# SensorsINI/v2e

Hardware: NVIDIA H100
Metric: Mevents/s (higher is better)
Workload: dtype fp16 tensor-core convs (fp32 accumulate) + f64 pixel state

## Files before the change

### include/v2e_b200.h

```cpp
#ifndef V2E_B200_H
#define V2E_B200_H

#include <stdint.h>

#ifdef __cplusplus
extern "C" {
#endif

typedef enum V2eStatus {
    V2E_OK = 0,
    V2E_E_INVALID = -1,
    V2E_E_CUDA = -2,
    V2E_E_CAPACITY = -3,
    V2E_E_ITER_CAP = -4,
    V2E_E_STATE = -5,
    V2E_E_UNSUPPORTED = -6,
    V2E_E_FALLBACK = -7
} V2eStatus;

typedef enum V2eFrameDtype { V2E_U8 = 0, V2E_F32 = 1, V2E_F64 = 2 } V2eFrameDtype;

const char *v2e_last_error(void);
int v2e_version(void);
int v2e_abi_info(int *version, int *emu_cfg_size, int *frame_info_size, int *unet_weights_size);
// ... 139 lines not shown
int v2e_conv2d_lrelu_sm100(const void *x1_dev, int C1, const void *x2_dev, int C2,
                           const void *wgt_dev, const float *bias_dev, int Cout_pad, int KH, int KW,
                           int N, int H, int W, void *out_dev, int out_cstride, int out_mode,
                           int co_real, float slope, void *stream);

enum {
    V2E_CONV_TILE_AUTO = -1,
    V2E_CONV_TILE_LEGACY = 0,
    V2E_CONV_TILE_256x128 = 1,
    V2E_CONV_TILE_128x256 = 2
};
int v2e_conv2d_lrelu_sm100_tile(const void *x1_dev, int C1, const void *x2_dev, int C2,
                                const void *wgt_dev, const float *bias_dev, int Cout_pad, int KH, int KW,
                                int N, int H, int W, void *out_dev, int out_cstride, int out_mode,
                                int co_real, float slope, int tile, void *stream);
int v2e_conv_pick_tile(int C1, int C2, int Cout_pad, int KH, int KW, int N, int H, int W, int n_sms);

int v2e_conv2d_lrelu_sm100_strip(const void *x1_dev, int C1, const void *x2_dev, int C2,
                                 const void *wgt_row_dev, const float *bias_dev, int Cout_pad, int KH,
                                 int KW, int N, int H, int W, void *out_dev, int out_cstride,
                                 int out_mode, int co_real, float slope, void *stream);
int v2e_conv_strip_pick_kc(int C1, int C2, int Cout_pad, int KH, int KW, int W);

int v2e_conv2d_up2_lrelu_sm100(const void *x_low_dev, int C, const void *wgt_fold_dev, const void *wgt_plain_dev,
                               const float *bias_dev, int Cout_pad, int N, int H_out, int W_out, void *out_dev,
                               int out_cstride, float slope, void *stream);
int v2e_conv_up2_fold_weights(const float *w_host, int cout, int cin, int Cout_pad, int C_pad, void *out_host);
int v2e_conv_up2_supported_c(int C, int Cout_pad, int W_out);

typedef struct V2eUNetWeights {
    const float *w[23];
    const float *b[23];
} V2eUNetWeights;

typedef struct V2eSlomo V2eSlomo;

int v2e_slomo_create(int H, int W, int max_batch, const V2eUNetWeights *flow,
                     const V2eUNetWeights *interp, V2eSlomo **out);
int v2e_slomo_destroy(V2eSlomo *h);
int v2e_slomo_set_pairs(V2eSlomo *h, const uint8_t *frames_u8_dev, int B, void *stream);
int v2e_slomo_max_flow(V2eSlomo *h, float *max_speed_host, void *stream);
int v2e_slomo_interp(V2eSlomo *h, double t, uint8_t *out_u8_dev, float *out_f32_dev, void *stream);
int v2e_slomo_check_finite(V2eSlomo *h, int *nonfinite_host, void *stream);
int v2e_slomo_set_option(V2eSlomo *h, int option, int value);
int v2e_slomo_profile(V2eSlomo *h, int enable);
int v2e_slomo_profile_read(V2eSlomo *h, float *conv_ms, int *conv_launches, double *conv_flops, void *stream);
// ... 70 lines not shown
```

### v2e_b200/_lib.py

```python
import ctypes
import os

from . import build as _build

_LIB = None


class V2eEmuCfg(ctypes.Structure):
    _fields_ = [
        ("width", ctypes.c_int32), ("height", ctypes.c_int32),
        ("per_pixel_thres", ctypes.c_int32), ("hdr", ctypes.c_int32),
        ("pos_thres_nominal", ctypes.c_double), ("neg_thres_nominal", ctypes.c_double),
        ("cutoff_hz", ctypes.c_double), ("leak_rate_hz", ctypes.c_double),
        ("leak_jitter_fraction", ctypes.c_double), ("refractory_period_s", ctypes.c_double),
        ("shot_noise_rate_hz", ctypes.c_double), ("shot_inten_factor", ctypes.c_double),
        ("rng_mode", ctypes.c_int32), ("iter_cap", ctypes.c_int32),
        ("seed", ctypes.c_uint64),
        ("csdvs", ctypes.c_int32), ("max_frames_per_step", ctypes.c_int32),
        ("cs_tau_p_s", ctypes.c_double), ("cs_tau_h_s", ctypes.c_double),
        ("scidvs", ctypes.c_int32), ("photoreceptor_noise", ctypes.c_int32),
        ("rng_pixel_offset", ctypes.c_uint32), ("full_frame_px", ctypes.c_uint32),
        ("own_row0", ctypes.c_int32), ("own_rows", ctypes.c_int32),
        ("cs_halo_rows", ctypes.c_int32), ("reserved1", ctypes.c_int32),
    ]
# ... 57 lines not shown
    "v2e_emu_phase_count": (_i, [_vp, _vp, _i, _d, _d, _vp, _vp, _i, _u64, _u64, _vp]),
    "v2e_emu_phase_update": (_i, [_vp, _vp, _i, _d, _d, _vp, _vp, _u64, _u64, _vp]),
    "v2e_emu_max_n_dev": (_vp, [_vp]),
    "v2e_emu_cs_begin": (_i, [_vp, _vp, _i, _d, _d, _u64, _u64, ctypes.POINTER(_i), _vp]),
    "v2e_emu_cs_pack": (_i, [_vp, _vp]),
    "v2e_emu_cs_unpack_from": (_i, [_vp, _vp, _vp, _vp]),
    "v2e_emu_cs_send_dev": (_vp, [_vp]),
    "v2e_emu_cs_chunk": (_i, [_vp, _i, _i, _vp]),
    "v2e_emu_cs_max_dev": (_vp, [_vp]),
    "v2e_emu_cs_advance": (_i, [_vp, _i, _i, _vp]),
    "v2e_emu_cs_update": (_i, [_vp, _vp, _i, _vp, _vp, _vp]),
    "v2e_emu_phase_filter": (_i, [_vp, _d, _d, _u64, _i, _vp]),
    "v2e_emu_read_counts": (_i, [_vp, ctypes.POINTER(ctypes.c_int32), _vp, _i, _vp]),
    "v2e_emu_phase_shot": (_i, [_vp, _vp, _i, _d, _d, _vp, _u64, _vp]),
    "v2e_emu_phase_emit": (_i, [_vp, _d, _d, _vp, _u64, _vp]),
    "v2e_conv2d_lrelu_sm100": (_i, [_vp, _i, _vp, _i, _vp, _vp, _i, _i, _i, _i, _i, _i, _vp, _i, _i, _i,
                                    ctypes.c_float, _vp]),
    "v2e_conv2d_lrelu_sm100_tile": (_i, [_vp, _i, _vp, _i, _vp, _vp, _i, _i, _i, _i, _i, _i, _vp, _i, _i, _i,
                                         ctypes.c_float, _i, _vp]),
    "v2e_conv_pick_tile": (_i, [_i, _i, _i, _i, _i, _i, _i, _i, _i]),
    "v2e_conv2d_lrelu_sm100_strip": (_i, [_vp, _i, _vp, _i, _vp, _vp, _i, _i, _i, _i, _i, _i, _vp, _i, _i, _i,
                                          ctypes.c_float, _vp]),
    "v2e_conv_strip_pick_kc": (_i, [_i, _i, _i, _i, _i, _i]),
    "v2e_conv2d_up2_lrelu_sm100": (_i, [_vp, _i, _vp, _vp, _vp, _i, _i, _i, _i, _vp, _i, ctypes.c_float, _vp]),
    "v2e_conv_up2_fold_weights": (_i, [_vp, _i, _i, _i, _i, _vp]),
    "v2e_conv_up2_supported_c": (_i, [_i, _i, _i]),
    "v2e_slomo_create": (_i, [_i, _i, _i, _vp, _vp, ctypes.POINTER(_vp)]),
    "v2e_slomo_destroy": (_i, [_vp]),
    "v2e_slomo_set_pairs": (_i, [_vp, _vp, _i, _vp]),
    "v2e_slomo_max_flow": (_i, [_vp, ctypes.POINTER(ctypes.c_float), _vp]),
    "v2e_slomo_interp": (_i, [_vp, _d, _vp, _vp, _vp]),
    "v2e_slomo_set_option": (_i, [_vp, _i, _i]),
    "v2e_slomo_check_finite": (_i, [_vp, ctypes.POINTER(_i), _vp]),
    "v2e_slomo_profile": (_i, [_vp, _i]),
    "v2e_slomo_profile_read": (_i, [_vp, ctypes.POINTER(ctypes.c_float), ctypes.POINTER(_i),
                                    ctypes.POINTER(ctypes.c_double), _vp]),
    "v2e_slomo_profile_read_layers": (_i, [_vp, ctypes.POINTER(ctypes.c_float), ctypes.POINTER(_i),
                                           ctypes.POINTER(ctypes.c_double), ctypes.POINTER(ctypes.c_float),
                                           ctypes.POINTER(_i), ctypes.POINTER(ctypes.c_double), _vp]),
    "v2e_slomo_flow_ptr": (_vp, [_vp]),
    "v2e_slomo_intrp_ptr": (_vp, [_vp]),
    "v2e_slomo_buffer_ptr": (_vp, [_vp, _i, _i]),
    "v2e_slomo_layer_kernel": (_i, [_vp, _i, _i]),
    "v2e_resize_create": (_i, [_i, _i, _i, _i, _i, _i, ctypes.POINTER(_vp)]),
    "v2e_resize_destroy": (_i, [_vp]),
    "v2e_resize_run": (_i, [_vp, _vp, _vp, _i, _vp]),
# ... 91 lines not shown
```

### v2e_b200/csrc/conv_tc.cu

```cuda
#include <cuda.h>
#include <cuda_fp16.h>
#include <cuda_runtime.h>
#include <math.h>
#include <stdint.h>
#include <stdio.h>
#include <string.h>
#include <vector>

#include "../../include/v2e_b200.h"
#include "common.cuh"
#include "tc_common.cuh"

namespace {

constexpr int kTileH = 8, kTileW = 16, kBM = kTileH * kTileW;
constexpr int kStages = 4;
constexpr int kConvThreads = 288;
constexpr int kProducerWarp = 8;
constexpr int kConsumerWarps = 8;

struct ConvParams {
    int N, H, W;
    int C1, C2;
    int KH, KW;
// ... 255 lines not shown
constexpr int kStripThreads = 288;

struct RowRing {
    uint64_t *full, *empty;
    uint32_t nslot, cnt;
    int waited, released;
    __device__ __forceinline__ uint32_t slot(int i) const { return (cnt + (uint32_t)i) % nslot; }
    __device__ __forceinline__ void wait_upto(int n) {
        for (; waited < n; waited++) {
            const uint32_t g = cnt + (uint32_t)waited;
            mbar_wait(&full[g % nslot], (g / nslot) & 1u);
        }
    }
    __device__ __forceinline__ void release_upto(int n, int lane) {
        wait_upto(n);
        __syncwarp();
        for (; released < n; released++)
            if (lane == 0) mbar_arrive(&empty[slot(released)]);
    }
};

template <int KW, int KC, int BN>
__device__ __forceinline__ void strip_pair_mma(float (&acc)[2][BN / 2], const RowRing &rr, int row0, int last, int slabs,
                                               uint64_t dr, uint64_t dw, uint32_t a_off, uint32_t row16, uint32_t slab16) {
    constexpr int KH = KW, taps = KH * KW;
    constexpr uint32_t rowb16 = (KC * 2u) >> 4, tile16 = (BN * KC * 2u) >> 4;
#pragma unroll
    for (int k = 0; k < 2; k++) {
#pragma unroll
        for (int i = 0; i < BN / 2; i++) acc[k][i] = 0.f;
        wgmma_fence_regs(acc[k]);
    }
    wgmma_fence();
#pragma unroll
    for (int rp = 0; rp <= KH; rp++) {
        const uint32_t a_row = rr.slot(row0 + (rp < KH ? rp : last)) * row16 + a_off;
        int sl = 0;
#pragma unroll 1
        do {
            const uint32_t a_lo = a_row + (uint32_t)sl * slab16;
#pragma unroll
            for (int s = 0; s < KW; s++) {
#pragma unroll
                for (int j = 0; j < KC / 16; j++) {
                    const uint64_t ad = desc_add(dr, a_lo + (uint32_t)s * rowb16 + 2u * j);
                    if (rp < KH) wgmma_f16<BN>(acc[0], ad, desc_add(dw, (uint32_t)(sl * taps + rp * KW + s) * tile16 + 2u * j), 1u);
                    if (rp > 0) wgmma_f16<BN>(acc[1], ad, desc_add(dw, (uint32_t)(sl * taps + (rp - 1) * KW + s) * tile16 + 2u * j), 1u);
                }
            }
        } while (++sl < slabs);
    }
    wgmma_commit();
}

template <int KW, int KC, int BN, bool POOL>
__global__ void __launch_bounds__(kStripThreads, 1)
conv_strip_kernel(const __grid_constant__ CUtensorMap tmA, const __grid_constant__ CUtensorMap tmA2,
                  const __grid_constant__ CUtensorMap tmB, const StripParams p) {
    extern __shared__ __align__(1024) uint8_t smem_raw[];
    uint8_t *smem = align1024(smem_raw);
    __shared__ __align__(8) uint64_t full_bar[kMaxSlot], empty_bar[kMaxSlot], w_bar;

    constexpr int KH = KW, ph = KH / 2, pw = KW / 2, taps = KH * KW;
    constexpr int PW = kRowTile + KW - 1;
    constexpr uint32_t tile_bytes = BN * KC * 2;
    const int warp = threadIdx.x >> 5, lane = threadIdx.x & 31;
    const int slabs = (p.C1 + p.C2) / KC;
    const uint32_t row_bytes = (uint32_t)p.slab_bytes * slabs;
    uint8_t *ring = smem + ((p.w_bytes + 1023) & ~1023);
    const int split = (int)blockIdx.x % p.n_split, co_off = split * BN;
    const int item0 = (int)blockIdx.x / p.n_split, item_step = (int)gridDim.x / p.n_split;

    if (threadIdx.x == 0) {
        for (int s = 0; s < p.nslot; s++) { mbar_init(&full_bar[s], 1); mbar_init(&empty_bar[s], kConsumerWarps); }
        mbar_init(&w_bar, 1);
        fence_barrier_init();
    }
    if (warp == kProducerWarp && lane == 0) {
        prefetch_tmap(&tmA);
        if (p.C2) prefetch_tmap(&tmA2);
        prefetch_tmap(&tmB);
    }
    __syncthreads();

    if (warp == kProducerWarp) {
        if (lane == 0) {
            mbar_expect_tx(&w_bar, (uint32_t)p.w_bytes);
            for (int t = 0; t < slabs * taps; t++)
                tma_load_2d(smem + (size_t)t * tile_bytes, &tmB, &w_bar, 0, t * p.cout_pad + co_off);
            uint32_t cnt = 0;
            for (int item = item0; item < p.n_items; item += item_step) {
                const int tx = item % p.tiles_x, rest = item / p.tiles_x;
                const int seg = rest % p.n_seg, n = rest / p.n_seg;
                const int ya = seg * p.seg_h, yb = min(p.H, ya + p.seg_h);
                const int x0 = tx * kRowTile;
                for (int i = ya - ph; i < yb + ph; i++, cnt++) {
                    const int slot = (int)(cnt % (uint32_t)p.nslot);
                    mbar_wait(&empty_bar[slot], ((cnt / (uint32_t)p.nslot) & 1u) ^ 1u);
                    mbar_expect_tx(&full_bar[slot], (uint32_t)(PW * KC * 2 * slabs));
                    uint8_t *dst = ring + (size_t)slot * row_bytes;
                    for (int sl = 0; sl < slabs; sl++) {
                        const int c = sl * KC;
                        if (c < p.C1) tma_load_4d(dst + (size_t)sl * p.slab_bytes, &tmA, &full_bar[slot], c, x0 - pw, i, n);
                        else tma_load_4d(dst + (size_t)sl * p.slab_bytes, &tmA2, &full_bar[slot], c - p.C1, x0 - pw, i, n);
                    }
                }
            }
        }
    } else {
        const int g = __shfl_sync(0xffffffffu, warp >> 2, 0);
        constexpr uint32_t sbo = 8u * KC * 2u, half16 = (64u * KC * 2u) >> 4;
        constexpr bool kOverlap = BN <= 32;
        const uint64_t dw = make_smem_desc(smem_u32(smem), swizzle_layout(KC), sbo);
        const uint64_t dr = make_smem_desc(smem_u32(ring), swizzle_layout(KC), sbo);
        const uint32_t row16 = row_bytes >> 4, slab16 = (uint32_t)p.slab_bytes >> 4;
        mbar_wait(&w_bar, 0);
        RowRing rr{full_bar, empty_bar, (uint32_t)p.nslot, 0u, 0, 0};
        for (int item = item0; item < p.n_items; item += item_step) {
            const int tx = item % p.tiles_x, rest = item / p.tiles_x;
            const int seg = rest % p.n_seg, n = rest / p.n_seg;
            const int ya = seg * p.seg_h, yb = min(p.H, ya + p.seg_h);
            const int rows_out = yb - ya, rows_in = rows_out + 2 * ph;
            rr.waited = 0; rr.released = 0;
            for (int q = g; 2 * q < rows_out; q += 2) {
                rr.release_upto(2 * q, lane);
                const bool two = 2 * q + 1 < rows_out;
                rr.wait_upto(2 * q + KH + (two ? 1 : 0));
                float acc[2][2][BN / 2];
                auto issue = [&](int hf) {
                    strip_pair_mma<KW, KC, BN>(acc[hf], rr, 2 * q, two ? KH : KH - 1, slabs, dr, dw, hf * half16, row16, slab16);
                };
                const int y = ya + 2 * q;
                auto epilogue = [&](int hf) {
#pragma unroll
                    for (int i = 0; i < 2; i++) {
                        const int m = 64 * hf + 16 * (warp & 3) + (lane >> 2) + 8 * i;
                        const int px = tx * kRowTile + m;
                        const bool inb = px < p.W;
                        const size_t pix = ((size_t)n * p.H + y) * p.W + px;
                        __half2 h0[BN / 8], h1[BN / 8];
                        epilogue_row<BN>(acc[hf][0], i, inb, pix, lane, p.bias + co_off, p.slope, p.out_mode, p.out,
                                         p.out_cstride, co_off, h0);
                        if (two) {
                            epilogue_row<BN>(acc[hf][1], i, inb, pix + p.W, lane, p.bias + co_off, p.slope, p.out_mode, p.out,
                                             p.out_cstride, co_off, h1);
                            if (POOL) {
                                __half2 *pl = (__half2 *)((__half *)p.pool_out +
                                    (((size_t)n * (p.H / 2) + y / 2) * (p.W / 2) + px / 2) * p.pool_cstride + co_off);
#pragma unroll
                                for (int j = 0; j < BN / 8; j++) {
                                    const float2 a = __half22float2(h1[j]), b = __half22float2(h0[j]);
                                    float s0 = a.x + b.x, s1 = a.y + b.y;
                                    s0 += __shfl_xor_sync(0xffffffffu, s0, 4);
                                    s1 += __shfl_xor_sync(0xffffffffu, s1, 4);
                                    if (inb && (lane & 4) == 0)
                                        pl[(8 * j + 2 * (lane & 3)) / 2] = __floats2half2_rn(s0 * 0.25f, s1 * 0.25f);
                                }
                            }
                        }
                    }
                };
                if constexpr (kOverlap) {
                    issue(0);
                    issue(1);
                    wgmma_wait<1>();
                    wgmma_fence_regs(acc[0][0]);
                    wgmma_fence_regs(acc[0][1]);
                    epilogue(0);
                    wgmma_wait<0>();
                    wgmma_fence_regs(acc[1][0]);
                    wgmma_fence_regs(acc[1][1]);
                    rr.release_upto(min(rows_in, 2 * q + 4), lane);
                    epilogue(1);
                } else {
#pragma unroll
                    for (int hf = 0; hf < 2; hf++) {
                        issue(hf);
                        wgmma_wait<0>();
                        wgmma_fence_regs(acc[hf][0]);
                        wgmma_fence_regs(acc[hf][1]);
                        if (hf == 1) rr.release_upto(min(rows_in, 2 * q + 4), lane);
                        epilogue(hf);
                    }
                }
            }
            rr.release_upto(rows_in, lane);
            rr.cnt += (uint32_t)rows_in;
        }
    }
}

constexpr int kUpBlocks = 6;

__global__ void __launch_bounds__(kStripThreads, 1)
conv_up2_kernel(const __grid_constant__ CUtensorMap tmA, const __grid_constant__ CUtensorMap tmB, const StripParams p) {
    constexpr int KC = 64, KW = 3, BN = 32;
    constexpr int PW = kRowTile + KW - 1;
    extern __shared__ __align__(1024) uint8_t smem_raw[];
    uint8_t *smem = align1024(smem_raw);
    __shared__ __align__(8) uint64_t full_bar[kMaxSlot], empty_bar[kMaxSlot], w_bar;

    const int warp = threadIdx.x >> 5, lane = threadIdx.x & 31;
    const int slabs = p.C1 / KC;
// ... 357 lines not shown

extern "C" int v2e_conv2d_lrelu_sm100_tile(const void *x1_dev, int C1, const void *x2_dev, int C2,
                                           const void *wgt_dev, const float *bias_dev, int Cout_pad, int KH, int KW,
                                           int N, int H, int W, void *out_dev, int out_cstride, int out_mode,
                                           int co_real, float slope, int tile, void *stream) {
    V2eConvLaunch L;
    int rc = v2e_conv_prepare(&L, x1_dev, C1, x2_dev, C2, wgt_dev, bias_dev, Cout_pad, KH, KW, N, H, W, out_dev,
                              out_cstride, out_mode, co_real, slope, tile, device_sms());
    if (rc) return rc;
    return v2e_conv_launch(&L, (cudaStream_t)stream);
}

extern "C" int v2e_conv2d_lrelu_sm100(const void *x1_dev, int C1, const void *x2_dev, int C2,
                                      const void *wgt_dev, const float *bias_dev, int Cout_pad, int KH, int KW,
                                      int N, int H, int W, void *out_dev, int out_cstride, int out_mode,
                                      int co_real, float slope, void *stream) {
    return v2e_conv2d_lrelu_sm100_tile(x1_dev, C1, x2_dev, C2, wgt_dev, bias_dev, Cout_pad, KH, KW, N, H, W, out_dev,
                                       out_cstride, out_mode, co_real, slope, V2E_CONV_TILE_AUTO, stream);
}

struct V2eStripLaunch {
    CUtensorMap tmA, tmA2, tmB;
    StripParams p;
    int grid;
    size_t smem;
};

static int make_rowseg_tmap(CUtensorMap *tm, const void *ptr, int N, int H, int W, int C, int KC, int KW) {
    EncodeTiledFn fn = encode_fn();
    if (!fn) return v2e_set_error(V2E_E_CUDA, "cuTensorMapEncodeTiled unavailable%s", "");
    cuuint64_t dims[4] = {(cuuint64_t)C, (cuuint64_t)W, (cuuint64_t)H, (cuuint64_t)N};
    cuuint64_t strides[3] = {(cuuint64_t)C * 2, (cuuint64_t)W * C * 2, (cuuint64_t)H * W * C * 2};
    cuuint32_t box[4] = {(cuuint32_t)KC, (cuuint32_t)(kRowTile + KW - 1), 1, 1};
    cuuint32_t es[4] = {1, 1, 1, 1};
    CUresult r = fn(tm, CU_TENSOR_MAP_DATA_TYPE_FLOAT16, 4, (void *)ptr, dims, strides, box, es,
                    CU_TENSOR_MAP_INTERLEAVE_NONE, swizzle_for(KC), CU_TENSOR_MAP_L2_PROMOTION_L2_256B,
                    CU_TENSOR_MAP_FLOAT_OOB_FILL_NONE);
    if (r != CUDA_SUCCESS) return v2e_set_error(V2E_E_CUDA, "cuTensorMapEncodeTiled failed for a strip row map%s", "");
    return V2E_OK;
}

constexpr size_t kSmemFull = 222 * 1024, kSmemHalf = 110 * 1024;

static int strip_config(int C1, int C2, int Cout_pad, int KH, int KW, int kc, int *nslot, int *ctas_per_sm, int *n_split) {
    if (Cout_pad > 64) return 0;
    const int slabs = (C1 + C2) / kc;
    const size_t row = (((size_t)(kRowTile + KW - 1) * kc * 2 + 1023) & ~(size_t)1023) * slabs;
    for (int split = 1; split <= 2; split++) {
        const int bn = Cout_pad / split;
        if (bn < 16 || bn % 16) break;
        const size_t wb = ((size_t)slabs * KH * KW * bn * kc * 2 + 1023) & ~(size_t)1023;
        const int two = wb + 2048 + (size_t)(KH + 3) * row <= kSmemHalf;
        const size_t budget = two ? kSmemHalf : kSmemFull;
        if (wb + 2048 + (size_t)(KH + 1) * row > budget) continue;
        int ns = (int)((budget - wb - 2048) / row);
        if (ns > kMaxSlot) ns = kMaxSlot;
        *nslot = ns; *ctas_per_sm = two ? 2 : 1; *n_split = split;
        return 1;
    }
    return 0;
}

constexpr int kStripMinW = 2 * kRowTile;

int v2e_strip_pick(int C1, int C2, int Cout_pad, int KH, int KW, int W, int *nslot_out) {
    if (Cout_pad > 64 || KH != KW || W < kStripMinW || (KW != 3 && KW != 5 && KW != 7)) return 0;
    const int g = C2 ? (C1 < C2 ? C1 : C2) : C1;
    const int kc = g % 64 == 0 ? 64 : (g % 32 == 0 ? 32 : 16);
    int ns, cps, nsp;
    if (!strip_config(C1, C2, Cout_pad, KH, KW, kc, &ns, &cps, &nsp)) return 0;
    if (nslot_out) *nslot_out = ns;
    return kc;
}

size_t v2e_strip_launch_size(void) { return sizeof(V2eStripLaunch); }

int v2e_strip_pool_supported(int C1, int C2, int Cout_pad, int KH, int KW, int H, int W) {
    if ((H & 1) || (W & 1) || Cout_pad < 32) return 0;
    const int KC = v2e_strip_pick(C1, C2, Cout_pad, KH, KW, W, nullptr);
    if (!((KW == 7 && KC == 32) || (KW == 5 && KC == 64))) return 0;
    int ns, cps, nsp;
    if (!strip_config(C1, C2, Cout_pad, KH, KW, KC, &ns, &cps, &nsp)) return 0;
    return cps == 1 && Cout_pad / nsp >= 32;
}

int v2e_strip_prepare(V2eStripLaunch *L, const void *x1, int C1, const void *x2, int C2, const void *wgt_row,
                      const float *bias, int Cout_pad, int KH, int KW, int N, int H, int W, void *out,
                      int out_cstride, int out_mode, int co_real, float slope, int n_sms, void *pool_out,
                      int pool_cstride) {
    memset(L, 0, sizeof(*L));
    StripParams &p = L->p;
    const int KC = v2e_strip_pick(C1, C2, Cout_pad, KH, KW, W, nullptr);
    int nslot = 0, ctas_per_sm = 0, n_split = 0;
    if (!KC || !strip_config(C1, C2, Cout_pad, KH, KW, KC, &nslot, &ctas_per_sm, &n_split))
        return v2e_set_error(V2E_E_INVALID, "layer does not qualify for the strip kernel%s", "");
    p.N = N; p.H = H; p.W = W; p.C1 = C1; p.C2 = C2; p.KH = KH; p.KW = KW; p.KC = KC;
    p.n_split = n_split; p.cout_pad = Cout_pad; p.BN = Cout_pad / n_split;
    p.tiles_x = (W + kRowTile - 1) / kRowTile;
    int seg_h = H;
    const int strips = p.tiles_x * N;
    while (seg_h > 4 * KH && (long)strips * ((H + seg_h - 1) / seg_h) < 6L * n_sms) seg_h = (seg_h + 1) / 2;
    if (pool_out) {
        if (out_mode != 0 || !v2e_strip_pool_supported(C1, C2, Cout_pad, KH, KW, H, W))
            return v2e_set_error(V2E_E_UNSUPPORTED, "strip: this layer has no pooled epilogue%s", "");
        seg_h = (seg_h + 1) & ~1;
    }
    p.pool_out = pool_out;
    p.pool_cstride = pool_cstride;
    p.seg_h = seg_h;
    p.n_seg = (H + seg_h - 1) / seg_h;
    p.n_items = strips * p.n_seg;
    p.nslot = nslot;
    const int slabs = (C1 + C2) / KC, taps = KH * KW;
    p.slab_bytes = (int)(((size_t)(kRowTile + KW - 1) * KC * 2 + 1023) & ~(size_t)1023);
    p.w_bytes = slabs * taps * p.BN * KC * 2;
    p.out_cstride = out_cstride; p.out_mode = out_mode; p.co_real = co_real; p.slope = slope;
    p.bias = bias; p.out = out;
    int rc;
    if ((rc = make_rowseg_tmap(&L->tmA, x1, N, H, W, C1, KC, KW))) return rc;
    if (C2) { if ((rc = make_rowseg_tmap(&L->tmA2, x2, N, H, W, C2, KC, KW))) return rc; }
    else L->tmA2 = L->tmA;
    {
        EncodeTiledFn fn = encode_fn();
        const int rows_total = slabs * taps * Cout_pad;
        cuuint64_t dims[2] = {(cuuint64_t)KC, (cuuint64_t)rows_total};
        cuuint64_t strides[1] = {(cuuint64_t)KC * 2};
        cuuint32_t box[2] = {(cuuint32_t)KC, (cuuint32_t)p.BN};
        cuuint32_t es[2] = {1, 1};
        CUresult r = fn(&L->tmB, CU_TENSOR_MAP_DATA_TYPE_FLOAT16, 2, (void *)wgt_row, dims, strides, box, es,
                        CU_TENSOR_MAP_INTERLEAVE_NONE, swizzle_for(KC), CU_TENSOR_MAP_L2_PROMOTION_L2_256B,
                        CU_TENSOR_MAP_FLOAT_OOB_FILL_NONE);
        if (r != CUDA_SUCCESS) return v2e_set_error(V2E_E_CUDA, "cuTensorMapEncodeTiled failed for strip weights%s", "");
    }
    L->smem = (size_t)((p.w_bytes + 1023) & ~1023) + (size_t)p.nslot * p.slab_bytes * slabs + 1024;
    int per = ctas_per_sm * n_sms / p.n_split;
    if (per > p.n_items) per = p.n_items;
    if (per < 1) per = 1;
    L->grid = per * p.n_split;
    return V2E_OK;
}

template <int KW, int KC, int BN, bool POOL>
static cudaError_t strip_launch_t(const V2eStripLaunch *L, cudaStream_t st) {
    static PerDeviceOnce attr_once;
    if (attr_once.first())
        cudaFuncSetAttribute(conv_strip_kernel<KW, KC, BN, POOL>, cudaFuncAttributeMaxDynamicSharedMemorySize, 226 * 1024);
    conv_strip_kernel<KW, KC, BN, POOL><<<L->grid, kStripThreads, L->smem, st>>>(L->tmA, L->tmA2, L->tmB, L->p);
    return cudaGetLastError();
}

template <int KW, int KC>
static int strip_launch_kc(const V2eStripLaunch *L, cudaStream_t st, cudaError_t *e) {
    const StripParams &p = L->p;
    if (p.KW != KW || p.KC != KC) return 0;
    if (p.pool_out) {
        if constexpr ((KW == 7 && KC == 32) || (KW == 5 && KC == 64)) {
            if (p.BN == 32) { *e = strip_launch_t<KW, KC, 32, true>(L, st); return 1; }
            if (p.BN == 64) { *e = strip_launch_t<KW, KC, 64, true>(L, st); return 1; }
        }
        return 0;
    }
    if (p.BN == 16) { *e = strip_launch_t<KW, KC, 16, false>(L, st); return 1; }
    if (p.BN == 32) { *e = strip_launch_t<KW, KC, 32, false>(L, st); return 1; }
    if (p.BN == 64) { *e = strip_launch_t<KW, KC, 64, false>(L, st); return 1; }
    return 0;
}

int v2e_strip_launch(const V2eStripLaunch *L, cudaStream_t st) {
    cudaError_t e = cudaSuccess;
    const int launched = strip_launch_kc<3, 16>(L, st, &e) || strip_launch_kc<3, 32>(L, st, &e) ||
                         strip_launch_kc<3, 64>(L, st, &e) || strip_launch_kc<5, 16>(L, st, &e) ||
                         strip_launch_kc<5, 32>(L, st, &e) || strip_launch_kc<5, 64>(L, st, &e) ||
                         strip_launch_kc<7, 16>(L, st, &e) || strip_launch_kc<7, 32>(L, st, &e) ||
                         strip_launch_kc<7, 64>(L, st, &e);
    if (!launched) return v2e_set_error(V2E_E_UNSUPPORTED, "strip kernel: unsupported filter width / slab / pooled epilogue%s", "");
    if (e != cudaSuccess) return v2e_set_error(V2E_E_CUDA, "conv_strip_kernel launch: %s", cudaGetErrorString(e));
    return V2E_OK;
}

extern "C" int v2e_conv2d_lrelu_sm100_strip(const void *x1_dev, int C1, const void *x2_dev, int C2,
                                            const void *wgt_row_dev, const float *bias_dev, int Cout_pad, int KH,
                                            int KW, int N, int H, int W, void *out_dev, int out_cstride,
                                            int out_mode, int co_real, float slope, void *stream) {
    V2eStripLaunch L;
    int dev = 0, sms = 132;
    cudaGetDevice(&dev);
    cudaDeviceGetAttribute(&sms, cudaDevAttrMultiProcessorCount, dev);
    int rc = v2e_strip_prepare(&L, x1_dev, C1, x2_dev, C2, wgt_row_dev, bias_dev, Cout_pad, KH, KW, N, H, W,
                               out_dev, out_cstride, out_mode, co_real, slope, sms, nullptr, 0);
    if (rc) return rc;
    return v2e_strip_launch(&L, (cudaStream_t)stream);
}


struct V2eUpLaunch {
    CUtensorMap tmA, tmB;
    StripParams p;
    int grid;
    size_t smem;
    const __half *low;
    const __half *w_plain;
    int C;
};

int v2e_conv_up2_supported(int C, int Cout_pad, int W_out) {
    if (C != 64 || Cout_pad != 32 || W_out % 2 || W_out < 2 * kStripMinW) return 0;
    const size_t wb = (size_t)(C / 64) * 2 * 3 * kUpBlocks * Cout_pad * 64 * 2;
    const size_t slab = ((size_t)(kRowTile + 2) * 64 * 2 + 1023) & ~(size_t)1023;
    return wb + 2048 + 3 * slab * (C / 64) <= kSmemFull;
}

extern "C" int v2e_conv_up2_fold_weights(const float *w, int cout, int cin, int Cout_pad, int C_pad, void *out_host) {
    if (!w || !out_host || C_pad % 64 || cin > C_pad || cout > Cout_pad) return v2e_set_error(V2E_E_INVALID, "bad argument%s", "");
    __half *o = (__half *)out_host;
// ... 111 lines not shown
```

### v2e_b200/csrc/slomo.cu

```cuda
#include <cuda.h>
#include <cuda_fp16.h>
#include <cuda_runtime.h>
#include <math.h>
#include <stdint.h>
#include <stdio.h>
#include <string.h>

#include <vector>

#include "../../include/v2e_b200.h"
#include "common.cuh"

struct V2eConvLaunch;
int v2e_conv_prepare(V2eConvLaunch *L, const void *x1, int C1, const void *x2, int C2, const void *wgt,
                     const float *bias, int Cout_pad, int KH, int KW, int N, int H, int W, void *out,
                     int out_cstride, int out_mode, int co_real, float slope, int tile, int n_sms);
int v2e_conv_launch(const V2eConvLaunch *L, cudaStream_t st);
size_t v2e_conv_launch_size(void);
struct V2eStripLaunch;
int v2e_strip_pick(int C1, int C2, int Cout_pad, int KH, int KW, int W, int *nslot_out);
size_t v2e_strip_launch_size(void);
int v2e_strip_pool_supported(int C1, int C2, int Cout_pad, int KH, int KW, int H, int W);
int v2e_strip_prepare(V2eStripLaunch *L, const void *x1, int C1, const void *x2, int C2, const void *wgt_row,
                      const float *bias, int Cout_pad, int KH, int KW, int N, int H, int W, void *out,
                      int out_cstride, int out_mode, int co_real, float slope, int n_sms, void *pool_out,
                      int pool_cstride);
int v2e_strip_launch(const V2eStripLaunch *L, cudaStream_t st);
struct V2eUpLaunch;
int v2e_conv_up2_supported(int C, int Cout_pad, int W_out);
extern "C" int v2e_conv_up2_fold_weights(const float *w, int cout, int cin, int Cout_pad, int C_pad, void *out_host);
size_t v2e_conv_up2_launch_size(void);
int v2e_conv_up2_prepare(V2eUpLaunch *L, const void *x_low, int C, const void *wgt_fold, const void *wgt_plain,
                         const float *bias, int Cout_pad, int N, int H, int W, void *out, int out_cstride, float slope,
                         int n_sms);
int v2e_conv_up2_launch(const V2eUpLaunch *L, cudaStream_t st);
int v2e_set_error(int code, const char *fmt, const char *detail);

#define CU(call)                                                                              \
    do {                                                                                      \
        cudaError_t e_ = (call);                                                              \
        if (e_ != cudaSuccess) return v2e_set_error(V2E_E_CUDA, #call ": %s", cudaGetErrorString(e_)); \
    } while (0)

namespace {

constexpr float kMean = 0.428f;
constexpr float kSlope = 0.1f;

__global__ void prep_pairs_kernel(const uint8_t *__restrict__ frames, float *__restrict__ img,
// ... 397 lines not shown
        for (int i = 0; i < 23; i++) { if (u->w[i]) cudaFree(u->w[i]); if (u->b[i]) cudaFree(u->b[i]); if (u->w_row[i]) cudaFree(u->w_row[i]); if (u->w_fold[i]) cudaFree(u->w_fold[i]); }
    void *ptrs[] = {h->in16, h->x0, h->s1, h->flow_out, h->intrp_out, h->img, h->maxspeed, h->nonfinite};
    for (void *p : ptrs) if (p) cudaFree(p);
    for (int l = 0; l < 5; l++) {
        cudaFree(h->pool[l]); cudaFree(h->da[l]); cudaFree(h->s[l]);
        cudaFree(h->up[l]); cudaFree(h->ua[l]); cudaFree(h->ub[l]);
    }
    for (cudaEvent_t e : h->ev) cudaEventDestroy(e);
    delete h;
    return V2E_OK;
}

static int conv(V2eSlomo *h, const UNet &u, int li, const __half *x1, const __half *x2, int B, int H, int W, void *out,
                int out_mode, cudaStream_t st, __half *pool_out = nullptr) {
    int rc;
    const bool row = u.row_kc[li] != 0;
    V2eConvLaunch *L = (V2eConvLaunch *)h->launch_mem.data();
    V2eStripLaunch *R = (V2eStripLaunch *)h->row_mem.data();
    h->ran[&u == &h->interp][li] = row ? (pool_out ? V2E_SLOMO_KERNEL_STRIP_POOL : V2E_SLOMO_KERNEL_STRIP)
                                       : V2E_SLOMO_KERNEL_TAP;
    if (row)
        rc = v2e_strip_prepare(R, x1, u.c1p[li], x2, x2 ? u.c2p[li] : 0, u.w_row[li], u.b[li], u.cout_pad[li], u.L[li].k,
                               u.L[li].k, B, H, W, out, u.cout_pad[li], out_mode, u.L[li].cout, kSlope, h->n_sms,
                               pool_out, u.cout_pad[li]);
    else
        rc = v2e_conv_prepare(L, x1, u.c1p[li], x2, x2 ? u.c2p[li] : 0, u.w[li], u.b[li], u.cout_pad[li], u.L[li].k,
                              u.L[li].k, B, H, W, out, u.cout_pad[li], out_mode, u.L[li].cout, kSlope,
                              V2E_CONV_TILE_AUTO, h->n_sms);
    if (rc) return rc;
    if (h->profile) {
        if (h->ev_used + 2 > h->ev.size()) {
            size_t old = h->ev.size();
            h->ev.resize(old + 512);
            for (size_t i = old; i < h->ev.size(); i++) cudaEventCreate(&h->ev[i]);
        }
        cudaEventRecord(h->ev[h->ev_used], st);
    }
    rc = row ? v2e_strip_launch(R, st) : v2e_conv_launch(L, st);
    if (h->profile) {
        cudaEventRecord(h->ev[h->ev_used + 1], st);
        h->ev_used += 2;
        const LayerSpec &l = u.L[li];
        const double fl = 2.0 * B * H * W * (double)l.cout * (l.cin1 + l.cin2) * l.k * l.k;
        h->conv_flops += fl;
        h->ev_layer.push_back(li);
        h->ev_flops.push_back(fl);
    }
// ... 280 lines not shown
```

### v2e_b200/csrc/tc_common.cuh

```cuda
#pragma once
#include <cuda.h>
#include <cuda_runtime.h>
#include <stdint.h>

__device__ __forceinline__ uint32_t smem_u32(const void *p) { return (uint32_t)__cvta_generic_to_shared(p); }

__device__ __forceinline__ void mbar_init(uint64_t *bar, uint32_t count) {
    asm volatile("mbarrier.init.shared::cta.b64 [%0], %1;" ::"r"(smem_u32(bar)), "r"(count) : "memory");
}
__device__ __forceinline__ void fence_barrier_init() { asm volatile("fence.mbarrier_init.release.cluster;" ::: "memory"); }
__device__ __forceinline__ void mbar_expect_tx(uint64_t *bar, uint32_t bytes) {
    asm volatile("mbarrier.arrive.expect_tx.shared::cta.b64 _, [%0], %1;" ::"r"(smem_u32(bar)), "r"(bytes) : "memory");
}
__device__ __forceinline__ void mbar_arrive(uint64_t *bar) {
    asm volatile("mbarrier.arrive.shared::cta.b64 _, [%0];" ::"r"(smem_u32(bar)) : "memory");
}
__device__ __forceinline__ void mbar_wait(uint64_t *bar, uint32_t parity) {
    const uint32_t addr = smem_u32(bar);
    uint32_t done;
    do {
        asm volatile(
            "{\n\t.reg .pred p;\n\t"
            "mbarrier.try_wait.parity.shared::cta.b64 p, [%1], %2;\n\t"
            "selp.u32 %0, 1, 0, p;\n\t}"
            : "=r"(done) : "r"(addr), "r"(parity) : "memory");
    } while (!done);
}

__device__ __forceinline__ void prefetch_tmap(const CUtensorMap *tm) {
    asm volatile("prefetch.tensormap [%0];" ::"l"((uint64_t)tm) : "memory");
}
__device__ __forceinline__ void tma_load_4d(void *dst, const CUtensorMap *tm, uint64_t *bar, int c0, int c1, int c2, int c3) {
    asm volatile(
// ... 80 lines not shown
```

Baseline: 55.29.

## Add stacked-weight wgmma chain for strip conv and split commit groups

Adds a 'stacked' weight layout for the row-strip conv kernel. Weight tiles are placed in shared memory with zero-padded gaps so that one wgmma with N=2*BN produces both output rows at once, replacing the paired per-row accumulators. It also splits the overlapped MMA issue into separate commit groups so input ring slots can be released earlier. An auto heuristic enables stacking only when BN<=32 and occupancy is unchanged. The cost is extra weight shared memory, a zero-fill at kernel start, and wasted MMA work on the zero tiles.

Measured after the change: 57.00 (median of 6 runs). +3.1%, better.

```diff
diff --git a/include/v2e_b200.h b/include/v2e_b200.h
--- a/include/v2e_b200.h
+++ b/include/v2e_b200.h
@@ -185,6 +185,17 @@
                                  int out_mode, int co_real, float slope, void *stream);
 int v2e_conv_strip_pick_kc(int C1, int C2, int Cout_pad, int KH, int KW, int W);
 
+enum {
+    V2E_STRIP_CHAIN_AUTO = -1,
+    V2E_STRIP_CHAIN_PAIRED = 0,
+    V2E_STRIP_CHAIN_STACKED = 1
+};
+int v2e_conv2d_lrelu_sm100_strip_chain(const void *x1_dev, int C1, const void *x2_dev, int C2,
+                                       const void *wgt_row_dev, const float *bias_dev, int Cout_pad, int KH,
+                                       int KW, int N, int H, int W, void *out_dev, int out_cstride,
+                                       int out_mode, int co_real, float slope, int chain, void *stream);
+int v2e_conv_strip_pick_chain(int C1, int C2, int Cout_pad, int KH, int KW, int W);
+
 int v2e_conv2d_up2_lrelu_sm100(const void *x_low_dev, int C, const void *wgt_fold_dev, const void *wgt_plain_dev,
                                const float *bias_dev, int Cout_pad, int N, int H_out, int W_out, void *out_dev,
                                int out_cstride, float slope, void *stream);
diff --git a/v2e_b200/_lib.py b/v2e_b200/_lib.py
--- a/v2e_b200/_lib.py
+++ b/v2e_b200/_lib.py
@@ -103,6 +103,9 @@
     "v2e_conv2d_lrelu_sm100_strip": (_i, [_vp, _i, _vp, _i, _vp, _vp, _i, _i, _i, _i, _i, _i, _vp, _i, _i, _i,
                                           ctypes.c_float, _vp]),
     "v2e_conv_strip_pick_kc": (_i, [_i, _i, _i, _i, _i, _i]),
+    "v2e_conv2d_lrelu_sm100_strip_chain": (_i, [_vp, _i, _vp, _i, _vp, _vp, _i, _i, _i, _i, _i, _i, _vp, _i, _i, _i,
+                                                ctypes.c_float, _i, _vp]),
+    "v2e_conv_strip_pick_chain": (_i, [_i, _i, _i, _i, _i, _i]),
     "v2e_conv2d_up2_lrelu_sm100": (_i, [_vp, _i, _vp, _vp, _vp, _i, _i, _i, _i, _vp, _i, ctypes.c_float, _vp]),
     "v2e_conv_up2_fold_weights": (_i, [_vp, _i, _i, _i, _i, _vp]),
     "v2e_conv_up2_supported_c": (_i, [_i, _i, _i]),
diff --git a/v2e_b200/csrc/conv_tc.cu b/v2e_b200/csrc/conv_tc.cu
--- a/v2e_b200/csrc/conv_tc.cu
+++ b/v2e_b200/csrc/conv_tc.cu
@@ -301,18 +301,12 @@
 
 template <int KW, int KC, int BN>
 __device__ __forceinline__ void strip_pair_mma(float (&acc)[2][BN / 2], const RowRing &rr, int row0, int last, int slabs,
-                                               uint64_t dr, uint64_t dw, uint32_t a_off, uint32_t row16, uint32_t slab16) {
+                                                uint64_t dr, uint64_t dw, uint32_t a_off, uint32_t row16, uint32_t slab16,
+                                                int rp0, int rp1) {
     constexpr int KH = KW, taps = KH * KW;
     constexpr uint32_t rowb16 = (KC * 2u) >> 4, tile16 = (BN * KC * 2u) >> 4;
 #pragma unroll
-    for (int k = 0; k < 2; k++) {
-#pragma unroll
-        for (int i = 0; i < BN / 2; i++) acc[k][i] = 0.f;
-        wgmma_fence_regs(acc[k]);
-    }
-    wgmma_fence();
-#pragma unroll
-    for (int rp = 0; rp <= KH; rp++) {
+    for (int rp = rp0; rp < rp1; rp++) {
         const uint32_t a_row = rr.slot(row0 + (rp < KH ? rp : last)) * row16 + a_off;
         int sl = 0;
 #pragma unroll 1
@@ -329,10 +323,39 @@
             }
         } while (++sl < slabs);
     }
-    wgmma_commit();
-}
-
-template <int KW, int KC, int BN, bool POOL>
+}
+
+template <int KW>
+__device__ __forceinline__ constexpr int stack_tiles() { return KW * (KW + 1) + 1; }
+template <int KW>
+__device__ __forceinline__ constexpr int stack_index(int r, int s) { return s * (KW + 1) + KW - r; }
+
+template <int KW, int KC, int BN>
+__device__ __forceinline__ void strip_stack_mma(float (&acc)[BN], const RowRing &rr, int row0, int last, int slabs,
+                                                 uint64_t dr, uint64_t dw, uint32_t a_off, uint32_t row16, uint32_t slab16,
+                                                 int rp0, int rp1) {
+    constexpr int KH = KW;
+    constexpr uint32_t rowb16 = (KC * 2u) >> 4, tile16 = (BN * KC * 2u) >> 4, wslab16 = stack_tiles<KW>() * tile16;
+#pragma unroll
+    for (int rp = rp0; rp < rp1; rp++) {
+        const uint32_t a_row = rr.slot(row0 + (rp < KH ? rp : last)) * row16 + a_off;
+        int sl = 0;
+#pragma unroll 1
+        do {
+            const uint32_t a_lo = a_row + (uint32_t)sl * slab16;
+            const uint32_t w_lo = (uint32_t)sl * wslab16 + (uint32_t)stack_index<KW>(rp, 0) * tile16;
+#pragma unroll
+            for (int s = 0; s < KW; s++) {
+#pragma unroll
+                for (int j = 0; j < KC / 16; j++)
+                    wgmma_f16<2 * BN>(acc, desc_add(dr, a_lo + (uint32_t)s * rowb16 + 2u * j),
+                                      desc_add(dw, w_lo + (uint32_t)(s * (KH + 1)) * tile16 + 2u * j), 1u);
+            }
+        } while (++sl < slabs);
+    }
+}
+
+template <int KW, int KC, int BN, bool POOL, bool STACK>
 __global__ void __launch_bounds__(kStripThreads, 1)
 conv_strip_kernel(const __grid_constant__ CUtensorMap tmA, const __grid_constant__ CUtensorMap tmA2,
                   const __grid_constant__ CUtensorMap tmB, const StripParams p) {
@@ -350,6 +373,15 @@
     const int split = (int)blockIdx.x % p.n_split, co_off = split * BN;
     const int item0 = (int)blockIdx.x / p.n_split, item_step = (int)gridDim.x / p.n_split;
 
+    if constexpr (STACK) {
+        constexpr int z_vec = (int)tile_bytes / 16, z_per_slab = KW + 1;
+        for (int i = threadIdx.x; i < slabs * z_per_slab * z_vec; i += blockDim.x) {
+            const int z = i / z_vec, sl = z / z_per_slab, s = z % z_per_slab;
+            ((uint4 *)(smem + ((size_t)sl * stack_tiles<KW>() + (size_t)s * (KH + 1)) * tile_bytes))[i % z_vec] =
+                make_uint4(0u, 0u, 0u, 0u);
+        }
+        fence_proxy_async();
+    }
     if (threadIdx.x == 0) {
         for (int s = 0; s < p.nslot; s++) { mbar_init(&full_bar[s], 1); mbar_init(&empty_bar[s], kConsumerWarps); }
         mbar_init(&w_bar, 1);
@@ -364,9 +396,12 @@
 
     if (warp == kProducerWarp) {
         if (lane == 0) {
-            mbar_expect_tx(&w_bar, (uint32_t)p.w_bytes);
-            for (int t = 0; t < slabs * taps; t++)
-                tma_load_2d(smem + (size_t)t * tile_bytes, &tmB, &w_bar, 0, t * p.cout_pad + co_off);
+            mbar_expect_tx(&w_bar, (uint32_t)(slabs * taps) * tile_bytes);
+            for (int t = 0; t < slabs * taps; t++) {
+                const int sl = t / taps, tap = t % taps;
+                const int dst = STACK ? sl * stack_tiles<KW>() + stack_index<KW>(tap / KW, tap % KW) : t;
+                tma_load_2d(smem + (size_t)dst * tile_bytes, &tmB, &w_bar, 0, t * p.cout_pad + co_off);
+            }
             uint32_t cnt = 0;
             for (int item = item0; item < p.n_items; item += item_step) {
                 const int tx = item % p.tiles_x, rest = item / p.tiles_x;
@@ -405,9 +440,20 @@
                 rr.release_upto(2 * q, lane);
                 const bool two = 2 * q + 1 < rows_out;
                 rr.wait_upto(2 * q + KH + (two ? 1 : 0));
-                float acc[2][2][BN / 2];
-                auto issue = [&](int hf) {
-                    strip_pair_mma<KW, KC, BN>(acc[hf], rr, 2 * q, two ? KH : KH - 1, slabs, dr, dw, hf * half16, row16, slab16);
+                float acc[2][BN];
+                auto rows = [&](int hf) -> float (&)[2][BN / 2] { return *reinterpret_cast<float (*)[2][BN / 2]>(acc[hf]); };
+                auto zero = [&](int hf) {
+#pragma unroll
+                    for (int i = 0; i < BN; i++) acc[hf][i] = 0.f;
+                    wgmma_fence_regs(acc[hf]);
+                };
+                auto issue = [&](int hf, int rp0, int rp1) {
+                    if constexpr (STACK)
+                        strip_stack_mma<KW, KC, BN>(acc[hf], rr, 2 * q, two ? KH : KH - 1, slabs, dr, dw, hf * half16,
+                                                     row16, slab16, rp0, rp1);
+                    else
+                        strip_pair_mma<KW, KC, BN>(rows(hf), rr, 2 * q, two ? KH : KH - 1, slabs, dr, dw, hf * half16,
+                                                    row16, slab16, rp0, rp1);
                 };
                 const int y = ya + 2 * q;
                 auto epilogue = [&](int hf) {
@@ -418,10 +464,10 @@
                         const bool inb = px < p.W;
                         const size_t pix = ((size_t)n * p.H + y) * p.W + px;
                         __half2 h0[BN / 8], h1[BN / 8];
-                        epilogue_row<BN>(acc[hf][0], i, inb, pix, lane, p.bias + co_off, p.slope, p.out_mode, p.out,
+                        epilogue_row<BN>(rows(hf)[0], i, inb, pix, lane, p.bias + co_off, p.slope, p.out_mode, p.out,
                                          p.out_cstride, co_off, h0);
                         if (two) {
-                            epilogue_row<BN>(acc[hf][1], i, inb, pix + p.W, lane, p.bias + co_off, p.slope, p.out_mode, p.out,
+                            epilogue_row<BN>(rows(hf)[1], i, inb, pix + p.W, lane, p.bias + co_off, p.slope, p.out_mode, p.out,
                                              p.out_cstride, co_off, h1);
                             if (POOL) {
                                 __half2 *pl = (__half2 *)((__half *)p.pool_out +
@@ -440,24 +486,34 @@
                     }
                 };
                 if constexpr (kOverlap) {
-                    issue(0);
-                    issue(1);
+                    zero(0);
+                    zero(1);
+                    wgmma_fence();
+                    issue(0, 0, 2);
+                    issue(1, 0, 2);
+                    wgmma_commit();
+                    issue(0, 2, KH + 1);
+                    wgmma_commit();
+                    issue(1, 2, KH + 1);
+                    wgmma_commit();
+                    wgmma_wait<2>();
+                    rr.release_upto(2 * q + 2, lane);
                     wgmma_wait<1>();
-                    wgmma_fence_regs(acc[0][0]);
-                    wgmma_fence_regs(acc[0][1]);
+                    wgmma_fence_regs(acc[0]);
                     epilogue(0);
                     wgmma_wait<0>();
-                    wgmma_fence_regs(acc[1][0]);
-                    wgmma_fence_regs(acc[1][1]);
+                    wgmma_fence_regs(acc[1]);
                     rr.release_upto(min(rows_in, 2 * q + 4), lane);
                     epilogue(1);
                 } else {
 #pragma unroll
                     for (int hf = 0; hf < 2; hf++) {
-                        issue(hf);
+                        zero(hf);
+                        wgmma_fence();
+                        issue(hf, 0, KH + 1);
+                        wgmma_commit();
                         wgmma_wait<0>();
-                        wgmma_fence_regs(acc[hf][0]);
-                        wgmma_fence_regs(acc[hf][1]);
+                        wgmma_fence_regs(acc[hf]);
                         if (hf == 1) rr.release_upto(min(rows_in, 2 * q + 4), lane);
                         epilogue(hf);
                     }
@@ -861,6 +917,7 @@
 struct V2eStripLaunch {
     CUtensorMap tmA, tmA2, tmB;
     StripParams p;
+    int stacked;
     int grid;
     size_t smem;
 };
@@ -881,14 +938,19 @@
 
 constexpr size_t kSmemFull = 222 * 1024, kSmemHalf = 110 * 1024;
 
-static int strip_config(int C1, int C2, int Cout_pad, int KH, int KW, int kc, int *nslot, int *ctas_per_sm, int *n_split) {
+static size_t strip_w_bytes(int slabs, int KH, int KW, int bn, int kc, int stacked) {
+    return (size_t)slabs * (stacked ? KW * (KH + 1) + 1 : KH * KW) * bn * kc * 2;
+}
+
+static int strip_config(int C1, int C2, int Cout_pad, int KH, int KW, int kc, int stacked, int *nslot, int *ctas_per_sm,
+                        int *n_split) {
     if (Cout_pad > 64) return 0;
     const int slabs = (C1 + C2) / kc;
     const size_t row = (((size_t)(kRowTile + KW - 1) * kc * 2 + 1023) & ~(size_t)1023) * slabs;
     for (int split = 1; split <= 2; split++) {
         const int bn = Cout_pad / split;
         if (bn < 16 || bn % 16) break;
-        const size_t wb = ((size_t)slabs * KH * KW * bn * kc * 2 + 1023) & ~(size_t)1023;
+        const size_t wb = (strip_w_bytes(slabs, KH, KW, bn, kc, stacked) + 1023) & ~(size_t)1023;
         const int two = wb + 2048 + (size_t)(KH + 3) * row <= kSmemHalf;
         const size_t budget = two ? kSmemHalf : kSmemFull;
         if (wb + 2048 + (size_t)(KH + 1) * row > budget) continue;
@@ -907,32 +969,57 @@
     const int g = C2 ? (C1 < C2 ? C1 : C2) : C1;
     const int kc = g % 64 == 0 ? 64 : (g % 32 == 0 ? 32 : 16);
     int ns, cps, nsp;
-    if (!strip_config(C1, C2, Cout_pad, KH, KW, kc, &ns, &cps, &nsp)) return 0;
+    if (!strip_config(C1, C2, Cout_pad, KH, KW, kc, 0, &ns, &cps, &nsp)) return 0;
     if (nslot_out) *nslot_out = ns;
     return kc;
 }
 
+static int strip_auto_stacked(int C1, int C2, int Cout_pad, int KH, int KW, int kc) {
+    int ns0, cps0, nsp0, ns1, cps1, nsp1;
+    if (!strip_config(C1, C2, Cout_pad, KH, KW, kc, 0, &ns0, &cps0, &nsp0) || Cout_pad / nsp0 > 32 ||
+        !strip_config(C1, C2, Cout_pad, KH, KW, kc, 1, &ns1, &cps1, &nsp1))
+        return 0;
+    return cps1 == cps0 && nsp1 == nsp0;
+}
+
+static int strip_plan(int C1, int C2, int Cout_pad, int KH, int KW, int kc, int chain, int *nslot, int *ctas_per_sm,
+                      int *n_split, int *stacked) {
+    *stacked = chain == V2E_STRIP_CHAIN_AUTO ? strip_auto_stacked(C1, C2, Cout_pad, KH, KW, kc)
+                                             : chain == V2E_STRIP_CHAIN_STACKED;
+    return strip_config(C1, C2, Cout_pad, KH, KW, kc, *stacked, nslot, ctas_per_sm, n_split);
+}
+
+extern "C" int v2e_conv_strip_pick_chain(int C1, int C2, int Cout_pad, int KH, int KW, int W) {
+    const int kc = v2e_strip_pick(C1, C2, Cout_pad, KH, KW, W, nullptr);
+    return kc ? strip_auto_stacked(C1, C2, Cout_pad, KH, KW, kc) : -1;
+}
+
 size_t v2e_strip_launch_size(void) { return sizeof(V2eStripLaunch); }
 
+static bool strip_pool_ok(int KW, int KC, int H, int W, int ctas_per_sm, int bn) {
+    return !(H & 1) && !(W & 1) && ((KW == 7 && KC == 32) || (KW == 5 && KC == 64)) && ctas_per_sm == 1 && bn >= 32;
+}
+
 int v2e_strip_pool_supported(int C1, int C2, int Cout_pad, int KH, int KW, int H, int W) {
-    if ((H & 1) || (W & 1) || Cout_pad < 32) return 0;
     const int KC = v2e_strip_pick(C1, C2, Cout_pad, KH, KW, W, nullptr);
-    if (!((KW == 7 && KC == 32) || (KW == 5 && KC == 64))) return 0;
-    int ns, cps, nsp;
-    if (!strip_config(C1, C2, Cout_pad, KH, KW, KC, &ns, &cps, &nsp)) return 0;
-    return cps == 1 && Cout_pad / nsp >= 32;
+    int ns, cps, nsp, st;
+    if (!KC || !strip_plan(C1, C2, Cout_pad, KH, KW, KC, V2E_STRIP_CHAIN_AUTO, &ns, &cps, &nsp, &st)) return 0;
+    return strip_pool_ok(KW, KC, H, W, cps, Cout_pad / nsp);
 }
 
 int v2e_strip_prepare(V2eStripLaunch *L, const void *x1, int C1, const void *x2, int C2, const void *wgt_row,
                       const float *bias, int Cout_pad, int KH, int KW, int N, int H, int W, void *out,
                       int out_cstride, int out_mode, int co_real, float slope, int n_sms, void *pool_out,
-                      int pool_cstride) {
+                      int pool_cstride, int chain) {
     memset(L, 0, sizeof(*L));
     StripParams &p = L->p;
+    if (chain < V2E_STRIP_CHAIN_AUTO || chain > V2E_STRIP_CHAIN_STACKED)
+        return v2e_set_error(V2E_E_INVALID, "strip: unknown chain%s", "");
     const int KC = v2e_strip_pick(C1, C2, Cout_pad, KH, KW, W, nullptr);
-    int nslot = 0, ctas_per_sm = 0, n_split = 0;
-    if (!KC || !strip_config(C1, C2, Cout_pad, KH, KW, KC, &nslot, &ctas_per_sm, &n_split))
-        return v2e_set_error(V2E_E_INVALID, "layer does not qualify for the strip kernel%s", "");
+    int nslot = 0, ctas_per_sm = 0, n_split = 0, stacked = 0;
+    if (!KC || !strip_plan(C1, C2, Cout_pad, KH, KW, KC, chain, &nslot, &ctas_per_sm, &n_split, &stacked))
+        return v2e_set_error(V2E_E_INVALID, "layer does not qualify for the strip kernel (with this chain)%s", "");
+    L->stacked = stacked;
     p.N = N; p.H = H; p.W = W; p.C1 = C1; p.C2 = C2; p.KH = KH; p.KW = KW; p.KC = KC;
     p.n_split = n_split; p.cout_pad = Cout_pad; p.BN = Cout_pad / n_split;
     p.tiles_x = (W + kRowTile - 1) / kRowTile;
@@ -940,7 +1027,7 @@
     const int strips = p.tiles_x * N;
     while (seg_h > 4 * KH && (long)strips * ((H + seg_h - 1) / seg_h) < 6L * n_sms) seg_h = (seg_h + 1) / 2;
     if (pool_out) {
-        if (out_mode != 0 || !v2e_strip_pool_supported(C1, C2, Cout_pad, KH, KW, H, W))
+        if (out_mode != 0 || !strip_pool_ok(KW, KC, H, W, ctas_per_sm, p.BN))
             return v2e_set_error(V2E_E_UNSUPPORTED, "strip: this layer has no pooled epilogue%s", "");
         seg_h = (seg_h + 1) & ~1;
     }
@@ -952,7 +1039,7 @@
     p.nslot = nslot;
     const int slabs = (C1 + C2) / KC, taps = KH * KW;
     p.slab_bytes = (int)(((size_t)(kRowTile + KW - 1) * KC * 2 + 1023) & ~(size_t)1023);
-    p.w_bytes = slabs * taps * p.BN * KC * 2;
+    p.w_bytes = (int)strip_w_bytes(slabs, KH, KW, p.BN, KC, stacked);
     p.out_cstride = out_cstride; p.out_mode = out_mode; p.co_real = co_real; p.slope = slope;
     p.bias = bias; p.out = out;
     int rc;
@@ -979,13 +1066,18 @@
     return V2E_OK;
 }
 
+template <int KW, int KC, int BN, bool POOL, bool STACK>
+static cudaError_t strip_launch_s(const V2eStripLaunch *L, cudaStream_t st) {
+    static PerDeviceOnce attr_once;
+    if (attr_once.first())
+        cudaFuncSetAttribute(conv_strip_kernel<KW, KC, BN, POOL, STACK>, cudaFuncAttributeMaxDynamicSharedMemorySize, 226 * 1024);
+    conv_strip_kernel<KW, KC, BN, POOL, STACK><<<L->grid, kStripThreads, L->smem, st>>>(L->tmA, L->tmA2, L->tmB, L->p);
+    return cudaGetLastError();
+}
+
 template <int KW, int KC, int BN, bool POOL>
 static cudaError_t strip_launch_t(const V2eStripLaunch *L, cudaStream_t st) {
-    static PerDeviceOnce attr_once;
-    if (attr_once.first())
-        cudaFuncSetAttribute(conv_strip_kernel<KW, KC, BN, POOL>, cudaFuncAttributeMaxDynamicSharedMemorySize, 226 * 1024);
-    conv_strip_kernel<KW, KC, BN, POOL><<<L->grid, kStripThreads, L->smem, st>>>(L->tmA, L->tmA2, L->tmB, L->p);
-    return cudaGetLastError();
+    return L->stacked ? strip_launch_s<KW, KC, BN, POOL, true>(L, st) : strip_launch_s<KW, KC, BN, POOL, false>(L, st);
 }
 
 template <int KW, int KC>
@@ -1017,18 +1109,26 @@
     return V2E_OK;
 }
 
-extern "C" int v2e_conv2d_lrelu_sm100_strip(const void *x1_dev, int C1, const void *x2_dev, int C2,
-                                            const void *wgt_row_dev, const float *bias_dev, int Cout_pad, int KH,
-                                            int KW, int N, int H, int W, void *out_dev, int out_cstride,
-                                            int out_mode, int co_real, float slope, void *stream) {
+extern "C" int v2e_conv2d_lrelu_sm100_strip_chain(const void *x1_dev, int C1, const void *x2_dev, int C2,
+                                                  const void *wgt_row_dev, const float *bias_dev, int Cout_pad, int KH,
+                                                  int KW, int N, int H, int W, void *out_dev, int out_cstride,
+                                                  int out_mode, int co_real, float slope, int chain, void *stream) {
     V2eStripLaunch L;
     int dev = 0, sms = 132;
     cudaGetDevice(&dev);
     cudaDeviceGetAttribute(&sms, cudaDevAttrMultiProcessorCount, dev);
     int rc = v2e_strip_prepare(&L, x1_dev, C1, x2_dev, C2, wgt_row_dev, bias_dev, Cout_pad, KH, KW, N, H, W,
-                               out_dev, out_cstride, out_mode, co_real, slope, sms, nullptr, 0);
+                               out_dev, out_cstride, out_mode, co_real, slope, sms, nullptr, 0, chain);
     if (rc) return rc;
     return v2e_strip_launch(&L, (cudaStream_t)stream);
+}
+
+extern "C" int v2e_conv2d_lrelu_sm100_strip(const void *x1_dev, int C1, const void *x2_dev, int C2,
+                                            const void *wgt_row_dev, const float *bias_dev, int Cout_pad, int KH,
+                                            int KW, int N, int H, int W, void *out_dev, int out_cstride,
+                                            int out_mode, int co_real, float slope, void *stream) {
+    return v2e_conv2d_lrelu_sm100_strip_chain(x1_dev, C1, x2_dev, C2, wgt_row_dev, bias_dev, Cout_pad, KH, KW, N, H, W,
+                                              out_dev, out_cstride, out_mode, co_real, slope, V2E_STRIP_CHAIN_AUTO, stream);
 }
 
 
diff --git a/v2e_b200/csrc/slomo.cu b/v2e_b200/csrc/slomo.cu
--- a/v2e_b200/csrc/slomo.cu
+++ b/v2e_b200/csrc/slomo.cu
@@ -24,7 +24,7 @@
 int v2e_strip_prepare(V2eStripLaunch *L, const void *x1, int C1, const void *x2, int C2, const void *wgt_row,
                       const float *bias, int Cout_pad, int KH, int KW, int N, int H, int W, void *out,
                       int out_cstride, int out_mode, int co_real, float slope, int n_sms, void *pool_out,
-                      int pool_cstride);
+                      int pool_cstride, int chain);
 int v2e_strip_launch(const V2eStripLaunch *L, cudaStream_t st);
 struct V2eUpLaunch;
 int v2e_conv_up2_supported(int C, int Cout_pad, int W_out);
@@ -468,7 +468,7 @@
     if (row)
         rc = v2e_strip_prepare(R, x1, u.c1p[li], x2, x2 ? u.c2p[li] : 0, u.w_row[li], u.b[li], u.cout_pad[li], u.L[li].k,
                                u.L[li].k, B, H, W, out, u.cout_pad[li], out_mode, u.L[li].cout, kSlope, h->n_sms,
-                               pool_out, u.cout_pad[li]);
+                               pool_out, u.cout_pad[li], V2E_STRIP_CHAIN_AUTO);
     else
         rc = v2e_conv_prepare(L, x1, u.c1p[li], x2, x2 ? u.c2p[li] : 0, u.w[li], u.b[li], u.cout_pad[li], u.L[li].k,
                               u.L[li].k, B, H, W, out, u.cout_pad[li], out_mode, u.L[li].cout, kSlope,
diff --git a/v2e_b200/csrc/tc_common.cuh b/v2e_b200/csrc/tc_common.cuh
--- a/v2e_b200/csrc/tc_common.cuh
+++ b/v2e_b200/csrc/tc_common.cuh
@@ -9,6 +9,7 @@
     asm volatile("mbarrier.init.shared::cta.b64 [%0], %1;" ::"r"(smem_u32(bar)), "r"(count) : "memory");
 }
 __device__ __forceinline__ void fence_barrier_init() { asm volatile("fence.mbarrier_init.release.cluster;" ::: "memory"); }
+__device__ __forceinline__ void fence_proxy_async() { asm volatile("fence.proxy.async.shared::cta;" ::: "memory"); }
 __device__ __forceinline__ void mbar_expect_tx(uint64_t *bar, uint32_t bytes) {
     asm volatile("mbarrier.arrive.expect_tx.shared::cta.b64 _, [%0], %1;" ::"r"(smem_u32(bar)), "r"(bytes) : "memory");
 }
```
